# TheStageAI/TheWhisper

Hardware: AMD Instinct MI355X
Metric: transcription tokens/sec (node), whisper-large-v3 10s chunks (higher is better)
Workload: dtype f16

## Files before the change

### thewhisper_amd/csrc/api.hip

```cpp
#include "../../include/thewhisper.h"
#include "tw_common.h"

#include <algorithm>
#include <cmath>
#include <cstdarg>
#include <cstdio>
#include <cstring>
#include <map>
#include <mutex>
#include <set>
#include <chrono>
#include <string>
#include <tuple>
#include <vector>

namespace {

thread_local std::string g_create_error;

struct LayerW {
  void *ln1_g = nullptr, *ln1_b = nullptr;
  void *wqkv = nullptr, *bqkv = nullptr;
  unsigned char *s_qkv = nullptr, *s_o = nullptr, *s_qc = nullptr, *s_oc = nullptr, *s_1 = nullptr, *s_2 = nullptr;
  void *wo = nullptr, *bo = nullptr;
// ... 11 lines not shown

struct tw_ctx {
  tw_config cfg{};
  int dtype = 1;
  bool w8 = false;
  int a16 = 0;
  bool fuse_cq = false;
  bool enc_fold = true;
  float *ln_stats_a = nullptr, *ln_stats_b = nullptr;
  float* du = nullptr;
  float* dstats = nullptr;
  unsigned char* logit_ws = nullptr;
  size_t esz = 2;
  int d = 0, H = 0, ffn = 0, V = 0, T = 0, Tp = 0, P = 0, C = 0, Bmax = 0, Le = 0, Ld = 0, n_mels = 0, Ha = 0;
  std::string err;
  std::vector<void*> allocs;
  hipStream_t own_stream = nullptr;

  void *conv1_w = nullptr, *conv1_b = nullptr, *conv2_w = nullptr, *conv2_b = nullptr;
  void *enc_pos_raw = nullptr, *enc_pos = nullptr, *enc_ln_g = nullptr, *enc_ln_b = nullptr;
  void *tok_emb = nullptr, *dec_pos = nullptr, *dec_ln_g = nullptr, *dec_ln_b = nullptr;
  void* logit_w = nullptr;
  float *logit_gw = nullptr, *logit_cb = nullptr;
  std::vector<LayerW> enc, dec;
  std::set<std::string> loaded;
  bool finalized = false;
  bool shares_weights = false;

  LogmelTables lm{};
  float* logspec_ws = nullptr; size_t logspec_cap = 0;
  unsigned* lm_max = nullptr;
  int* n_valid_dev = nullptr;

  void *melT = nullptr, *h1 = nullptr, *xa = nullptr, *xb = nullptr, *lnbuf = nullptr, *qbuf = nullptr, *kbuf = nullptr,
       *vtbuf = nullptr, *attn = nullptr, *ffnh = nullptr, *enc_out = nullptr;
  int encoded_B = 0, cross_B = 0;

  void *self_k = nullptr, *self_v = nullptr, *cross_k = nullptr, *cross_v = nullptr;
  unsigned char *cross_ksc = nullptr, *cross_vsc = nullptr;
  void *dx0 = nullptr, *dx1 = nullptr, *dq = nullptr, *datt = nullptr, *dh = nullptr;
  float* logits = nullptr;
  float* align = nullptr;
  int* align_slot = nullptr;
  int *seq = nullptr, *cur_ids = nullptr, *finished = nullptr, *last_ts = nullptr;
  DecState* stt = nullptr;
  int* begin_suppress_dev = nullptr; int* suppress_dev = nullptr;
  SamplerPartial* sampler_partials = nullptr;
  float* sample_inv_t = nullptr; uint32_t* sample_key = nullptr; uint32_t* sample_off = nullptr; int* sample_noisy = nullptr;
  SamplePartial* sample_parts = nullptr;
  int* filter_top_k = nullptr; float* filter_top_p = nullptr; int* filter_choice = nullptr;
  unsigned* suppress_bits = nullptr;
  int* h_pinned = nullptr;
  int* row_ids = nullptr;
  int* h_rows = nullptr;
  int* row_lastts = nullptr;
  int* row_choice = nullptr;
  int* verify_state = nullptr;
  int* h_verify = nullptr;
  int* bias_tab = nullptr; int* h_bias = nullptr;
  int* repeat_tab = nullptr; int* h_repeat = nullptr;
  int* n_pad_tab = nullptr; int* h_n_pad = nullptr;
  int last_draft[4] = {0, 0, 0, 0};
  size_t row_ids_cap = 0;
  int* score_seq = nullptr;
  int *score_bsup = nullptr, *score_sup = nullptr;
  unsigned* score_bits = nullptr;
  ScorePartial* score_parts = nullptr;
  float* score_out = nullptr;
  float* h_score = nullptr;
  int row_cap = 0;
  int* h_stage = nullptr;
  size_t h_stage_ints = 0;
  hipEvent_t ring_ev[8]{};
  int last_seq_len = 0, last_n_prompt = 0;
  int dec_key_bound = 0;
  int enc_pos_rows = 0;

  float *zbuf = nullptr, *mat = nullptr, *out_ts = nullptr;
  signed char* trace = nullptr;
  int* n_cols = nullptr;

  std::map<std::string, hipGraphExec_t> step_graphs;
  std::string step_graph_key;

  hipEvent_t ev0[5]{}, ev1[5]{};
  bool ev_valid[5]{};
  int last_steps = 0;
};

namespace {

int fail(tw_ctx* c, int code, const char* fmt, ...) {
  char buf[512];
  va_list ap;
  va_start(ap, fmt);
  vsnprintf(buf, sizeof buf, fmt, ap);
  va_end(ap);
  if (c) c->err = buf; else g_create_error = buf;
  return code;
}

#define HIPCHK(c, expr)                                                                       \
  do {                                                                                        \
    hipError_t _e = (expr);                                                                   \
    if (_e != hipSuccess)                                                                     \
      return fail((c), TW_EHIP, "%s failed: %s (%s:%d)", #expr, hipGetErrorString(_e), __FILE__, __LINE__); \
  } while (0)

template <typename P>
int dalloc(tw_ctx* c, P** p, size_t bytes, bool zero) {
  void* q = nullptr;
  if (bytes == 0) bytes = 16;
  hipError_t e = hipMalloc(&q, bytes);
  if (e != hipSuccess) return fail(c, TW_ENOMEM, "hipMalloc(%zu) failed: %s", bytes, hipGetErrorString(e));
  c->allocs.push_back(q);
  if (zero) {
    e = hipMemset(q, 0, bytes);
    if (e != hipSuccess) return fail(c, TW_EHIP, "hipMemset failed: %s", hipGetErrorString(e));
  }
  *p = reinterpret_cast<P*>(q);
  return TW_OK;
}
#define ALLOC(c, ptr, bytes, zero)                   \
  do {                                               \
    int _r = dalloc((c), &(ptr), (bytes), (zero));   \
    if (_r != TW_OK) return _r;                      \
  } while (0)

inline hipStream_t pick_stream(tw_ctx* c, void* s) { return s ? reinterpret_cast<hipStream_t>(s) : c->own_stream; }

struct DeviceGuard {
  int prev = -1;
  bool switched = false;
  explicit DeviceGuard(int dev) {
    if (hipGetDevice(&prev) == hipSuccess && prev != dev) switched = hipSetDevice(dev) == hipSuccess;
  }
  ~DeviceGuard() {
    if (switched) (void)hipSetDevice(prev);
  }
  DeviceGuard(const DeviceGuard&) = delete;
  DeviceGuard& operator=(const DeviceGuard&) = delete;
};
#define TW_ON_DEVICE(c) DeviceGuard _tw_guard((c)->cfg.device)

char* at(void* base, size_t elems, size_t esz) { return reinterpret_cast<char*>(base) + elems * esz; }

void build_mel_bank(int n_mels, std::vector<float>& bank, std::vector<int>& lo, std::vector<int>& hi) {
  const int nb = 201;
  auto hz2mel = [](double f) { return f >= 1000.0 ? 15.0 + std::log(f / 1000.0) * (27.0 / std::log(6.4)) : 3.0 * f / 200.0; };
  auto mel2hz = [](double m) { return m >= 15.0 ? 1000.0 * std::exp((std::log(6.4) / 27.0) * (m - 15.0)) : 200.0 * m / 3.0; };
  const double mmin = hz2mel(0.0), mmax = hz2mel(8000.0);
  std::vector<double> ff(n_mels + 2);
  for (int i = 0; i < n_mels + 2; ++i) ff[i] = mel2hz(mmin + (mmax - mmin) * (double)i / (double)(n_mels + 1));
  bank.assign((size_t)nb * n_mels, 0.f);
  lo.assign(n_mels, nb);
  hi.assign(n_mels, 0);
  for (int k = 0; k < nb; ++k) {
    const double fk = 8000.0 * (double)k / (double)(nb - 1);
    for (int m = 0; m < n_mels; ++m) {
      const double down = -(ff[m] - fk) / (ff[m + 1] - ff[m]);
      const double up = (ff[m + 2] - fk) / (ff[m + 2] - ff[m + 1]);
      double v = std::fmax(0.0, std::fmin(down, up));
      v *= 2.0 / (ff[m + 2] - ff[m]);
      const float vf = (float)v;
      bank[(size_t)k * n_mels + m] = vf;
      if (vf != 0.f) {
        if (k < lo[m]) lo[m] = k;
        if (k + 1 > hi[m]) hi[m] = k + 1;
      }
    }
  }
  for (int m = 0; m < n_mels; ++m)
    if (hi[m] == 0) lo[m] = 0;
}

int upload(tw_ctx* c, void* dst, const void* src, size_t bytes) {
  HIPCHK(c, hipMemcpy(dst, src, bytes, hipMemcpyHostToDevice));
  return TW_OK;
}

void tic(tw_ctx* c, int i, hipStream_t st) { (void)hipEventRecord(c->ev0[i], st); }
void toc(tw_ctx* c, int i, hipStream_t st) { (void)hipEventRecord(c->ev1[i], st); c->ev_valid[i] = true; }

}

extern "C" {

const char* tw_version(void) { return TW_VERSION_STRING; }

const char* tw_last_error(const tw_ctx* ctx) { return ctx ? ctx->err.c_str() : g_create_error.c_str(); }

int tw_destroy(tw_ctx* c) {
  if (!c) return TW_OK;
  TW_ON_DEVICE(c);
  (void)hipDeviceSynchronize();
  for (auto& kv : c->step_graphs) (void)hipGraphExecDestroy(kv.second);
  for (void* p : c->allocs) (void)hipFree(p);
  if (c->h_pinned) (void)hipHostFree(c->h_pinned);
  if (c->h_stage) (void)hipHostFree(c->h_stage);
  if (c->h_rows) (void)hipHostFree(c->h_rows);
  if (c->h_verify) (void)hipHostFree(c->h_verify);
  if (c->h_score) (void)hipHostFree(c->h_score);
  if (c->h_bias) (void)hipHostFree(c->h_bias);
  if (c->h_repeat) (void)hipHostFree(c->h_repeat);
  if (c->h_n_pad) (void)hipHostFree(c->h_n_pad);
  for (int i = 0; i < 5; ++i) {
    if (c->ev0[i]) (void)hipEventDestroy(c->ev0[i]);
    if (c->ev1[i]) (void)hipEventDestroy(c->ev1[i]);
  }
  for (int i = 0; i < 8; ++i)
    if (c->ring_ev[i]) (void)hipEventDestroy(c->ring_ev[i]);
  if (c->own_stream) (void)hipStreamDestroy(c->own_stream);
  delete c;
  return TW_OK;
}

static int create_ctx(const tw_config* cfg, const tw_ctx* share, tw_ctx** out);

int tw_create(const tw_config* cfg, tw_ctx** out) { return create_ctx(cfg, nullptr, out); }

int tw_create_sibling(const tw_ctx* src, int32_t max_batch, tw_ctx** out) {
  if (!src || !out) return fail(nullptr, TW_EINVAL, "tw_create_sibling: null argument");
  if (!src->finalized) return fail(nullptr, TW_ESTATE, "tw_create_sibling: the source context's weights are not finalized");
  if (src->shares_weights) return fail(nullptr, TW_EINVAL, "tw_create_sibling: the source is itself a sibling (create it from the owner)");
  tw_config cfg = src->cfg;
  cfg.max_batch = max_batch;
  return create_ctx(&cfg, src, out);
}

static int create_ctx(const tw_config* cfg, const tw_ctx* share, tw_ctx** out) {
  if (!cfg || !out) return fail(nullptr, TW_EINVAL, "tw_create: null argument");
  *out = nullptr;
  if (cfg->heads <= 0 || cfg->d_model != cfg->heads * 64)
    return fail(nullptr, TW_EINVAL, "head_dim must be 64 (d_model=%d heads=%d)", cfg->d_model, cfg->heads);
  if (cfg->dtype != TW_BF16 && cfg->dtype != TW_F32 && cfg->dtype != TW_F16 && cfg->dtype != TW_BF16_MXFP8 && cfg->dtype != TW_BF16_W8A16)
    return fail(nullptr, TW_EINVAL, "dtype must be TW_BF16, TW_F16, TW_F32, TW_BF16_MXFP8 or TW_BF16_W8A16");
  const bool cfg_w8 = cfg->dtype == TW_BF16_MXFP8 || cfg->dtype == TW_BF16_W8A16;
  if (cfg_w8 && (cfg->d_model % 128 || cfg->ffn % 128))
    return fail(nullptr, TW_EINVAL, "TW_BF16_MXFP8 / TW_BF16_W8A16 need d_model and ffn to be multiples of 128");
  if (cfg->d_model % 64 || cfg->ffn % 64 || cfg->d_model > 1280)
    return fail(nullptr, TW_EINVAL, "d_model/ffn must be multiples of 64 and d_model <= 1280");
  if (cfg->max_batch < 1 || cfg->max_batch > 64) return fail(nullptr, TW_EINVAL, "max_batch must be in [1,64]");
  if (cfg->dtype == TW_BF16_MXFP8 && cfg->max_batch > 16)
    return fail(nullptr, TW_EINVAL, "TW_BF16_MXFP8: max_batch must be in [1,16] (TW_BF16_W8A16 takes up to 64 streams)");
  if (cfg->source_positions < 8 || cfg->source_positions > 1500 || cfg->target_positions < 8 || cfg->target_positions > 511)
    return fail(nullptr, TW_EINVAL, "source_positions must be in [8,1500], target_positions in [8,511]");
  if (cfg->n_align_heads < 0 || cfg->n_align_heads > TW_MAX_ALIGN_HEADS) return fail(nullptr, TW_EINVAL, "bad n_align_heads");
  if (cfg->n_mels < 1 || cfg->n_mels > 256) return fail(nullptr, TW_EINVAL, "bad n_mels");
  int ndev = 0;
  if (hipGetDeviceCount(&ndev) != hipSuccess || ndev <= 0)
    return fail(nullptr, TW_EHIP, "no HIP device available (the MI355X path has no CPU fallback)");
  if (cfg->device < 0 || cfg->device >= ndev) return fail(nullptr, TW_EINVAL, "device %d out of range", cfg->device);
  DeviceGuard guard(cfg->device);
  int cur = -1;
  if (hipGetDevice(&cur) != hipSuccess || cur != cfg->device) return fail(nullptr, TW_EHIP, "hipSetDevice(%d) failed", cfg->device);

  tw_ctx* c = new tw_ctx();
  c->cfg = *cfg;
  c->w8 = cfg_w8;
  c->a16 = cfg->dtype == TW_BF16_W8A16;
  c->dtype = c->w8 ? (int)TW_BF16 : cfg->dtype;
  c->esz = c->dtype == TW_F32 ? 4 : 2;
  c->d = cfg->d_model; c->H = cfg->heads; c->ffn = cfg->ffn; c->V = cfg->vocab;
  c->T = cfg->source_positions; c->Tp = (c->T + 63) / 64 * 64; c->P = cfg->target_positions;
  c->n_mels = cfg->n_mels; c->C = (cfg->n_mels + 63) / 64 * 64;
  c->Bmax = cfg->max_batch; c->Le = cfg->enc_layers; c->Ld = cfg->dec_layers; c->Ha = cfg->n_align_heads;
  c->fuse_cq = c->d == c->H * 64;
  c->enc_fold = c->d % 64 == 0 && c->d <= 1280;
  auto bail = [&](int r) { g_create_error = c->err; tw_destroy(c); return r; };
#define CALLOC(ptr, bytes, zero) do { int _r = dalloc(c, &(ptr), (bytes), (zero)); if (_r != TW_OK) return bail(_r); } while (0)
#define CHIP(expr) do { hipError_t _e = (expr); if (_e != hipSuccess) { fail(c, TW_EHIP, "%s: %s", #expr, hipGetErrorString(_e)); return bail(TW_EHIP); } } while (0)
  CHIP(hipStreamCreate(&c->own_stream));
  for (int i = 0; i < 5; ++i) { CHIP(hipEventCreate(&c->ev0[i])); CHIP(hipEventCreate(&c->ev1[i])); }
  for (int i = 0; i < 8; ++i) CHIP(hipEventCreateWithFlags(&c->ring_ev[i], hipEventDisableTiming));
  CHIP(hipHostMalloc(reinterpret_cast<void**>(&c->h_pinned), sizeof(int) * (8 * 64 + 64 + 16), hipHostMallocDefault));
  c->h_stage_ints = (size_t)c->Bmax * c->P + 3 * (size_t)c->Bmax + 64 + 1024 + 16 + 6 * 64 + 2 * 64;
  CHIP(hipHostMalloc(reinterpret_cast<void**>(&c->h_stage), sizeof(int) * c->h_stage_ints, hipHostMallocDefault));

  const size_t e = c->esz;
// ... 542 lines not shown
bool getenv_off_fuse() {
  static const bool off = []() { const char* e = getenv("TW_FUSE_CQ"); return e && atoi(e) == 0; }();
  return off;
}

int decode_core(tw_ctx* c, int B, hipStream_t st, int rs = 0, const int* ids = nullptr, bool embed = true, bool rows_logits = false,
                bool record_alignment = true, const int* n_pad = nullptr) {
  const int d = c->d, H = c->H, F = c->ffn, T = c->T, P = c->P, dt = c->dtype;
  const size_t e = c->esz;
  if (n_pad && (rs != 0 || !embed)) return fail(c, TW_EINVAL, "decode_core: a ragged step is an ordinary step with its own embedding");
  if (n_pad) HIPCHK(c, launch_embed_ragged(dt, c->cur_ids, c->stt, n_pad, c->tok_emb, c->dec_pos, c->dx0, B, d, st));
  else if (embed) HIPCHK(c, launch_embed(dt, rs > 0 ? ids : c->cur_ids, c->stt, c->tok_emb, c->dec_pos, c->dx0, B, d, rs, st));
  void* xin = c->dx0;
  void* xmid = c->dx1;
  const int Pp = (P + 63) / 64 * 64;
  const size_t self_layer = (size_t)c->Bmax * Pp * d;
  const size_t cross_layer = (size_t)c->Bmax * c->Tp * d;
  for (int l = 0; l < c->Ld; ++l) {
    const LayerW& L = c->dec[l];
    void* sk = at(c->self_k, self_layer * l, e);
    void* sv = at(c->self_v, self_layer * l, e);
    const bool fq_on = c->fuse_cq && !getenv_off_fuse() && d / (L.tr_o ? L.tr_o : 16) <= 192;
    {
      GemvArgs a{};
      a.x = xin; a.ldx = d; a.ln_gw = L.qkv_gw; a.ln_cb = L.qkv_cb; a.W = L.wqkv; a.wscale = L.s_qkv; a.a16 = c->a16; a.N = (fq_on ? 4 : 3) * d; a.K = d; a.B = B;
      a.y = c->dq; a.ldy = d; a.kcache = sk; a.vcache = sv; a.cache_bstride = (long long)Pp * d; a.cache_hstride = (long long)Pp * 64; a.d_model = d; a.stt = c->stt;
      a.u = fq_on ? c->du : nullptr;
      a.rows_streams = rs;
      a.n_pad = n_pad;
      HIPCHK(c, launch_gemv(dt, a, st));
    }
    if (n_pad) HIPCHK(c, launch_dec_self_attn_ragged(dt, c->dq, sk, sv, Pp, c->datt, B, H, c->dec_key_bound > 0 ? c->dec_key_bound : P, c->stt, n_pad, st));
    else HIPCHK(c, launch_dec_self_attn(dt, c->dq, sk, sv, Pp, c->datt, B, H, c->dec_key_bound > 0 ? c->dec_key_bound : P, c->stt, rs, st));
    {
      GemvArgs a{};
      a.x = c->datt; a.ldx = d; a.W = L.wo; a.wscale = L.s_o; a.a16 = c->a16; a.tr = L.tr_o; a.bias = L.bo; a.N = (fq_on ? 2 : 1) * d; a.K = d; a.B = B;
      a.res = xin; a.ldres = d; a.y = xmid; a.ldy = d;
      if (fq_on) { a.u = c->du; a.nsplit = d; a.stats = c->dstats; }
      HIPCHK(c, launch_gemv(dt, a, st));
    }
    FusedQ fq{};
    if (fq_on) {
      fq.u = c->du; fq.stats = c->dstats; fq.n_part = d / (L.tr_o ? L.tr_o : 16); fq.gw = L.qc_gw; fq.cb = L.qc_cb; fq.d = d;
    } else {
      GemvArgs a{};
      a.x = xmid; a.ldx = d; a.ln_gw = L.qc_gw; a.ln_cb = L.qc_cb; a.W = L.wq_c; a.wscale = L.s_qc; a.a16 = c->a16; a.tr = L.tr_qc; a.N = d; a.K = d; a.B = B;
      a.y = c->dq; a.ldy = d;
      HIPCHK(c, launch_gemv(dt, a, st));
    }
    HIPCHK(c, launch_dec_cross_attn(dt, c->dq, fq, at(c->cross_k, cross_layer * l, c->w8 ? 1 : e), at(c->cross_v, cross_layer * l, c->w8 ? 1 : e),
                                    c->datt, B, H, T, c->Tp, (c->Ha > 0 && record_alignment) ? c->align_slot + (size_t)l * H : nullptr, c->align,
                                    record_alignment ? c->Ha : 0,
                                    P, c->stt, c->w8 ? c->cross_ksc + (size_t)c->Bmax * H * c->Tp * l : nullptr,
                                    c->w8 ? c->cross_vsc + (size_t)c->Bmax * H * c->Tp * l : nullptr, rs, st));
    {
      GemvArgs a{};
      a.x = c->datt; a.ldx = d; a.W = L.wo_c; a.wscale = L.s_oc; a.a16 = c->a16; a.tr = L.tr_oc; a.bias = L.bo_c; a.N = d; a.K = d; a.B = B; a.res = xmid; a.ldres = d;
      a.y = xin; a.ldy = d;
      HIPCHK(c, launch_gemv(dt, a, st));
    }
    {
      GemvArgs a{};
      a.x = xin; a.ldx = d; a.ln_gw = L.fc1_gw; a.ln_cb = L.fc1_cb; a.W = L.w1; a.wscale = L.s_1; a.a16 = c->a16; a.tr = L.tr_1; a.N = F; a.K = d; a.B = B;
      a.gelu = 1; a.y = c->dh; a.ldy = F;
      HIPCHK(c, launch_gemv(dt, a, st));
    }
    {
      GemvArgs a{};
      a.x = c->dh; a.ldx = F; a.W = L.w2; a.wscale = L.s_2; a.a16 = c->a16; a.tr = L.tr_2; a.bias = L.b2; a.N = d; a.K = F; a.B = B; a.res = xin; a.ldres = d;
      a.y = xmid; a.ldy = d;
      HIPCHK(c, launch_gemv(dt, a, st));
    }
    void* t = xin; xin = xmid; xmid = t;
  }
  if (rs == 0 || rows_logits) {
    GemvArgs a{};
    a.x = xin; a.ldx = d; a.ln_gw = c->logit_gw; a.ln_cb = c->logit_cb; a.W = c->logit_w; a.wscale = c->logit_ws; a.a16 = c->a16; a.N = c->V; a.K = d; a.B = B;
    a.y_f32 = c->logits;
    HIPCHK(c, launch_gemv(dt, a, st));
  }
  return TW_OK;
}

int prefill_core(tw_ctx* c, int B, const int* tok, int ld, int n_pos, hipStream_t st) {
  if (n_pos <= 0) return TW_OK;
  const int cap = (c->w8 && !c->a16) ? 16 : 64;
  if (B > cap) return fail(c, TW_EINVAL, "prefill: %d streams exceed the %d rows of a launch", B, cap);
  const int L = std::max(1, std::min(cap, c->row_cap) / B);
  if ((size_t)n_pos * B > c->row_ids_cap) return fail(c, TW_EINVAL, "prefill: %d positions x %d streams exceed the row table", n_pos, B);
  int* h = c->h_rows;
  for (int p = 0; p < n_pos; ++p)
    for (int b = 0; b < B; ++b) h[(size_t)p * B + b] = tok[(size_t)b * ld + p];
  HIPCHK(c, hipMemcpyAsync(c->row_ids, h, sizeof(int) * (size_t)n_pos * B, hipMemcpyHostToDevice, st));
  for (int p0 = 0; p0 < n_pos; p0 += L) {
    const int l = std::min(L, n_pos - p0);
    c->dec_key_bound = std::min(((p0 + l + 63) / 64) * 64, ((c->P + 63) / 64) * 64);
    int r = decode_core(c, l * B, st, B, c->row_ids + (size_t)p0 * B);
    if (r != TW_OK) return r;
    HIPCHK(c, launch_advance(c->stt, l, st));
  }
  return TW_OK;
}

int verify_round(tw_ctx* c, int B, int* tok, int ld, int n_begin, int ts_begin, int p_start, int p_end, int rows_cap, const SamplerArgs& sa0,
                 hipStream_t st, int* p_next, int* n_launches, int p_given, int* next_given, const SeqBiasArgs* ba,
                 const RepeatArgs* ra) {
  const int n_pos = p_end - p_start + 1;
  if (n_pos < 1 || B > rows_cap) return fail(c, TW_EINVAL, "verify: bad round [%d, %d] for %d streams", p_start, p_end, B);
  if ((size_t)n_pos * B > c->row_ids_cap) return fail(c, TW_EINVAL, "verify: %d positions x %d streams exceed the row table", n_pos, B);
  const int L = std::max(1, rows_cap / B);
  int* h = c->h_rows;
  int* hl = c->h_rows + c->row_ids_cap;
  for (int b = 0; b < B; ++b) {
    int lt = -1;
    for (int p = n_begin; p < p_start; ++p) if (tok[(size_t)b * ld + p] >= ts_begin) lt = tok[(size_t)b * ld + p];
    for (int p = p_start; p <= p_end; ++p) {
      const int t = tok[(size_t)b * ld + p];
      if (p >= n_begin && t >= ts_begin) lt = t;
      h[(size_t)(p - p_start) * B + b] = t;
      hl[(size_t)(p - p_start) * B + b] = lt;
    }
  }
  int* hv = c->h_verify;
  hv[66] = 0x7fffffff; hv[67] = 0;
  HIPCHK(c, hipMemcpyAsync(c->row_ids, h, sizeof(int) * (size_t)n_pos * B, hipMemcpyHostToDevice, st));
  HIPCHK(c, hipMemcpyAsync(c->row_lastts, hl, sizeof(int) * (size_t)n_pos * B, hipMemcpyHostToDevice, st));
  HIPCHK(c, hipMemcpyAsync(c->verify_state, hv + 66, sizeof(int) * 2, hipMemcpyHostToDevice, st));
  for (int p0 = p_start; p0 <= p_end; p0 += L) {
    const int l = std::min(L, p_end - p0 + 1);
    const size_t off = (size_t)(p0 - p_start) * B;
    c->dec_key_bound = std::min(((p0 + l + 63) / 64) * 64, ((c->P + 63) / 64) * 64);
    int r = decode_core(c, l * B, st, B, c->row_ids + off, true, true);
    if (r != TW_OK) return r;
    SamplerArgs sa = sa0;
    sa.B = l * B; sa.rows_streams = B; sa.row_pos0 = p0; sa.row_lastts = c->row_lastts + off; sa.row_choice = c->row_choice + off;
    sa.row_last_pos = p_end; sa.row_is_last = (p0 + l > p_end) ? 1 : 0; sa.verify_state = c->verify_state;
    if (ba) {
      SeqBiasArgs b = *ba;
      b.rows = l * B; b.rows_streams = B; b.row_pos0 = p0;
      HIPCHK(c, launch_seq_bias(b, st));
    }
    if (ra) {
      RepeatArgs rp = *ra;
      rp.rows = l * B; rp.rows_streams = B; rp.row_pos0 = p0;
      HIPCHK(c, launch_repeat(rp, st));
    }
    HIPCHK(c, launch_sampler_rows(sa, st));
    HIPCHK(c, hipMemcpyAsync(hv, c->verify_state, sizeof(int) * (2 + B), hipMemcpyDeviceToHost, st));
    HIPCHK(c, hipStreamSynchronize(st));
    ++*n_launches;
    if (hv[1] != 0) {
      const int pn = hv[1];
      if (pn < p0 + 1 || pn > p0 + l) return fail(c, TW_EHIP, "verify: decided position %d outside the launch [%d, %d)", pn - 1, p0, p0 + l);
      bool same = pn <= p_given;
      for (int b = 0; b < B; ++b) {
        same = same && tok[(size_t)b * ld + pn] == hv[2 + b];
        tok[(size_t)b * ld + pn] = hv[2 + b];
      }
      *next_given = same ? 1 : 0;
      *p_next = pn;
      return TW_OK;
    }
  }
  return fail(c, TW_EHIP, "verify: the round ended without a decision");
}

constexpr size_t kSeqBiasTabWords = kSeqBiasHeader + 2 * (size_t)TW_BIAS_MAX_SEQS + 2 * ((size_t)TW_BIAS_MAX_SEQS + 1) + TW_BIAS_MAX_TOKENS;

int pack_seq_bias(tw_ctx* c, int B, const tw_bias_opts* bo, std::vector<int>& tab) {
  const char* fn = "tw_generate_greedy_biased";
  const int S = bo->n_seq;
  if (S < 0 || S > TW_BIAS_MAX_SEQS) return fail(c, TW_EINVAL, "%s: %d sequences (at most %d)", fn, S, TW_BIAS_MAX_SEQS);
  if (!bo->row_off || !bo->seq_off || !bo->tokens || !bo->bias) return fail(c, TW_EINVAL, "%s: null array in tw_bias_opts", fn);
  if (bo->row_off[0] != 0 || bo->row_off[B] != S) return fail(c, TW_EINVAL, "%s: row_off must run from 0 to n_seq", fn);
  for (int b = 0; b < B; ++b)
    if (bo->row_off[b + 1] < bo->row_off[b]) return fail(c, TW_EINVAL, "%s: row_off decreases at row %d", fn, b);
  if (bo->seq_off[0] != 0) return fail(c, TW_EINVAL, "%s: seq_off must start at 0", fn);
  for (int i = 0; i < S; ++i) {
    const long long L = (long long)bo->seq_off[i + 1] - bo->seq_off[i];
    if (L < 1 || L > TW_BIAS_MAX_SEQ_LEN) return fail(c, TW_EINVAL, "%s: sequence %d has %lld tokens (1 .. %d)", fn, i, L, TW_BIAS_MAX_SEQ_LEN);
    if (bo->seq_off[i + 1] > TW_BIAS_MAX_TOKENS) return fail(c, TW_EINVAL, "%s: more than %d tokens", fn, TW_BIAS_MAX_TOKENS);
    if (!std::isfinite(bo->bias[i])) return fail(c, TW_EINVAL, "%s: the bias of sequence %d is NaN or infinite", fn, i);
  }
// ... 37 lines not shown
  auto append = [&](int slot, const int* p, size_t n) { tab[slot] = (int)tab.size(); tab.insert(tab.end(), p, p + n); };
  append(0, grp_off.data(), grp_off.size());
  append(1, grp_tok.data(), grp_tok.size());
  append(2, seq_off.data(), seq_off.size());
  append(3, reinterpret_cast<const int*>(bias.data()), bias.size());
  append(4, tokens.data(), tokens.size());
  if (tab.size() > kSeqBiasTabWords) return fail(c, TW_EINVAL, "%s: the packed table exceeds its capacity", fn);
  return TW_OK;
}

int pack_repeat(tw_ctx* c, const char* fn, int rows, int max_n, const tw_repeat_opts* ro, int* tab, bool* any) {
  if (rows < 1 || rows > 64) return fail(c, TW_EINVAL, "%s: %d rows (1..64)", fn, rows);
  if (ro->penalty_ignore < 0) return fail(c, TW_EINVAL, "%s: penalty_ignore %d < 0", fn, ro->penalty_ignore);
  *any = false;
  for (int b = 0; b < 64; ++b) {
    const float r = (b < rows && ro->penalty) ? ro->penalty[b] : 1.0f;
    const int N = (b < rows && ro->no_repeat_ngram) ? ro->no_repeat_ngram[b] : 0;
    if (!std::isfinite(r) || !(r > 0.f)) return fail(c, TW_EINVAL, "%s: the penalty of row %d is NaN, infinite or <= 0", fn, b);
    if (N < 0 || N > max_n) return fail(c, TW_EINVAL, "%s: no_repeat_ngram[%d] = %d outside [0, %d]", fn, b, N, max_n);
    memcpy(tab + b, &r, sizeof r);
    tab[64 + b] = N;
    *any |= r != 1.0f || N != 0;
  }
  tab[128] = ro->penalty_ignore;
  for (int i = 129; i < kRepeatTabWords; ++i) tab[i] = 0;
  return TW_OK;
}

int reset_state(tw_ctx* c, int n_prompt, hipStream_t st) {
  DecState s{0, n_prompt, 0, 0};
  memcpy(c->h_pinned + 576, &s, sizeof s);
  HIPCHK(c, hipMemcpyAsync(c->stt, c->h_pinned + 576, sizeof s, hipMemcpyHostToDevice, st));
  return TW_OK;
}

}

extern "C" {

int tw_decoder_reset(tw_ctx* c, int32_t B, void* stream) {
  if (!c) return TW_EINVAL;
  TW_ON_DEVICE(c);
  if (B < 1 || B > c->cross_B) return fail(c, TW_ESTATE, "tw_decoder_reset: B=%d but cross K/V holds %d clips", B, c->cross_B);
  hipStream_t st = pick_stream(c, stream);
  int r = reset_state(c, 0, st);
  if (r != TW_OK) return r;
  c->dec_key_bound = c->P;
  HIPCHK(c, hipStreamSynchronize(st));
  return TW_OK;
}

int tw_decode_step(tw_ctx* c, int32_t B, const int32_t* ids_host, float* logits_dev, void* stream) {
  if (!c || !ids_host) return fail(c, TW_EINVAL, "tw_decode_step: null argument");
  TW_ON_DEVICE(c);
  if (B < 1 || B > c->cross_B) return fail(c, TW_ESTATE, "tw_decode_step: B=%d but cross K/V holds %d clips", B, c->cross_B);
  hipStream_t st = pick_stream(c, stream);
  HIPCHK(c, hipMemcpyAsync(c->cur_ids, ids_host, sizeof(int) * B, hipMemcpyHostToDevice, st));
  int r = decode_core(c, B, st);
  if (r != TW_OK) return r;
  if (logits_dev)
    HIPCHK(c, hipMemcpyAsync(logits_dev, c->logits, sizeof(float) * (size_t)B * c->V, hipMemcpyDeviceToDevice, st));
  HIPCHK(c, launch_advance(c->stt, 1, st));
  return TW_OK;
}

static int generate_loop(tw_ctx* c, int32_t B, const int32_t* prompt, int32_t n_prompt, const tw_greedy_opts* o, const tw_sample_opts* so,
                         const tw_filter_opts* fo, const tw_bias_opts* bo, int32_t* out_ids, int32_t* out_len, void* stream,
                         const int32_t* n_pad = nullptr, const tw_repeat_opts* ro = nullptr) {
  const char* fn = n_pad ? "tw_generate_greedy_ragged" : ro ? "tw_generate_greedy_repeat" : bo ? "tw_generate_greedy_biased" : fo ? "tw_generate_sample_filtered" : so ? "tw_generate_sample" : "tw_generate_greedy";
  const bool ragged = n_pad != nullptr;
  if (ragged && (so || fo || bo || ro || o->n_forced != 0 || o->n_draft != 0)) return fail(c, TW_EINVAL, "%s: padding goes with the plain greedy call only", fn);
  if (B < 1 || B > c->cross_B) return fail(c, TW_ESTATE, "%s: B=%d but cross K/V holds %d clips", fn, B, c->cross_B);
  if (n_prompt < 1 || n_prompt >= c->P) return fail(c, TW_EINVAL, "bad n_prompt %d", n_prompt);
  if (o->n_begin_suppress > 64 || o->n_suppress > 1024) return fail(c, TW_EINVAL, "suppress lists too long");
  if (o->want_alignment && c->Ha == 0) return fail(c, TW_EINVAL, "want_alignment but the context has no alignment heads");
  const int n_forced = o->n_forced;
  if (n_forced < 0 || n_forced >= n_prompt) return fail(c, TW_EINVAL, "bad n_forced %d (n_prompt %d)", n_forced, n_prompt);
  const int n_draft = o->n_draft;
  if (n_draft < 0 || n_draft >= n_prompt || (n_draft > 0 && n_forced > 0))
    return fail(c, TW_EINVAL, "bad n_draft %d (n_prompt %d, n_forced %d: one of the two)", n_draft, n_prompt, n_forced);
  if (o->pad_id < 0 || o->pad_id >= c->V || o->eos_id < 0 || o->eos_id >= c->V)
    return fail(c, TW_EINVAL, "pad_id %d / eos_id %d outside the vocabulary", o->pad_id, o->eos_id);
  const int n_begin = n_prompt - n_forced - n_draft;
  int max_len = n_begin + o->max_new_tokens;
  if (o->max_length > 0 && o->max_length < max_len) max_len = o->max_length;
  if (max_len > c->P) max_len = c->P;
  if (max_len <= n_prompt) return fail(c, TW_EINVAL, "nothing to generate (max_len %d <= n_prompt %d)", max_len, n_prompt);
  const int out_ld = o->max_length > 0 ? o->max_length : max_len;
  const bool biased = bo != nullptr;
  std::vector<int> bias_tab;
  if (biased) {
    if (B > 64) return fail(c, TW_EINVAL, "%s: %d streams (1..64)", fn, B);
    int r = pack_seq_bias(c, B, bo, bias_tab);
    if (r != TW_OK) return r;
  }
  int repeat_tab[kRepeatTabWords];
  bool repeat = false;
  if (ro) {
    if (so || fo) return fail(c, TW_EINVAL, "%s: repeat options go with the greedy call only", fn);
    int r = pack_repeat(c, fn, B, c->P, ro, repeat_tab, &repeat);
    if (r != TW_OK) return r;
  }
  c->dec_key_bound = max_len;
  hipStream_t st = pick_stream(c, stream);
  const int P = c->P;

  int* hseq = c->h_stage;
  int* first = hseq + (size_t)c->Bmax * P;
  int* zeros = first + c->Bmax;
  int* neg = zeros + c->Bmax;
  int* bsup = neg + c->Bmax;
  int* sup = bsup + 64;
  DecState* s0p = reinterpret_cast<DecState*>(sup + 1024);
  float* h_inv_t = reinterpret_cast<float*>(sup + 1024 + 16);
  uint32_t* h_key = reinterpret_cast<uint32_t*>(h_inv_t + 64);
  uint32_t* h_off = h_key + 128;
  int* h_noisy = reinterpret_cast<int*>(h_off + 128);
  int* h_top_k = h_noisy + 64;
  float* h_top_p = reinterpret_cast<float*>(h_top_k + 64);
  for (size_t i = 0; i < (size_t)B * P; ++i) hseq[i] = o->pad_id;
  for (int b = 0; b < B; ++b) {
    for (int i = 0; i < n_prompt; ++i) {
      const int t = prompt[(size_t)b * n_prompt + i];
      if (t < 0 || t >= c->V) return fail(c, TW_EINVAL, "prompt token %d out of range", t);
      hseq[(size_t)b * P + i] = t;
    }
    first[b] = prompt[(size_t)b * n_prompt + (n_forced > 0 ? n_prompt - 1 : 0)];
    zeros[b] = (so && so->temperature[b] < 0.f) ? 1 : 0;
    neg[b] = -1;
    if (so) {
      const float t = so->temperature[b];
      h_noisy[b] = t > 0.f ? 1 : 0;
      h_inv_t[b] = t > 0.f ? 1.0f / t : 1.0f;
      const uint64_t sd = so->seed ? so->seed[b] : 0, of = so->offset ? so->offset[b] : 0;
      h_key[2 * b] = (uint32_t)sd; h_key[2 * b + 1] = (uint32_t)(sd >> 32);
      h_off[2 * b] = (uint32_t)of; h_off[2 * b + 1] = (uint32_t)(of >> 32);
      if (fo) {
        h_top_k[b] = (t > 0.f && fo->top_k) ? fo->top_k[b] : 0;
        h_top_p[b] = (t > 0.f && fo->top_p) ? fo->top_p[b] : 1.0f;
      }
    }
    for (int i = n_begin; i < n_prompt; ++i) {
      const int t = prompt[(size_t)b * n_prompt + i];
      if (t == o->eos_id) return fail(c, TW_EINVAL, n_draft > 0 ? "a draft token is <eos>" : "a forced token is <eos>");
      if (n_forced > 0 && o->timestamps && t > o->no_timestamps_id) neg[b] = t;
    }
  }
  if (biased) {
    if (!c->bias_tab) ALLOC(c, c->bias_tab, sizeof(int) * kSeqBiasTabWords, false);
    if (!c->h_bias) HIPCHK(c, hipHostMalloc(reinterpret_cast<void**>(&c->h_bias), sizeof(int) * kSeqBiasTabWords));
    memcpy(c->h_bias, bias_tab.data(), sizeof(int) * bias_tab.size());
    HIPCHK(c, hipMemcpyAsync(c->bias_tab, c->h_bias, sizeof(int) * bias_tab.size(), hipMemcpyHostToDevice, st));
  }
  if (repeat) {
    if (!c->repeat_tab) ALLOC(c, c->repeat_tab, sizeof(int) * kRepeatTabWords, true);
    if (!c->h_repeat) HIPCHK(c, hipHostMalloc(reinterpret_cast<void**>(&c->h_repeat), sizeof(int) * kRepeatTabWords));
    memcpy(c->h_repeat, repeat_tab, sizeof repeat_tab);
    HIPCHK(c, hipMemcpyAsync(c->repeat_tab, c->h_repeat, sizeof repeat_tab, hipMemcpyHostToDevice, st));
  }
  if (ragged) {
    if (!c->n_pad_tab) ALLOC(c, c->n_pad_tab, sizeof(int) * 64, true);
    if (!c->h_n_pad) HIPCHK(c, hipHostMalloc(reinterpret_cast<void**>(&c->h_n_pad), sizeof(int) * 64));
    for (int b = 0; b < 64; ++b) c->h_n_pad[b] = b < B ? n_pad[b] : 0;
    HIPCHK(c, hipMemcpyAsync(c->n_pad_tab, c->h_n_pad, sizeof(int) * 64, hipMemcpyHostToDevice, st));
  }
  HIPCHK(c, hipMemcpyAsync(c->seq, hseq, sizeof(int) * (size_t)B * P, hipMemcpyHostToDevice, st));
  HIPCHK(c, hipMemcpyAsync(c->cur_ids, first, sizeof(int) * B, hipMemcpyHostToDevice, st));
  HIPCHK(c, hipMemcpyAsync(c->finished, zeros, sizeof(int) * B, hipMemcpyHostToDevice, st));
  HIPCHK(c, hipMemcpyAsync(c->last_ts, neg, sizeof(int) * B, hipMemcpyHostToDevice, st));
  if (so) {
    HIPCHK(c, hipMemcpyAsync(c->sample_inv_t, h_inv_t, sizeof(float) * B, hipMemcpyHostToDevice, st));
    HIPCHK(c, hipMemcpyAsync(c->sample_key, h_key, sizeof(uint32_t) * 2 * B, hipMemcpyHostToDevice, st));
    HIPCHK(c, hipMemcpyAsync(c->sample_off, h_off, sizeof(uint32_t) * 2 * B, hipMemcpyHostToDevice, st));
    HIPCHK(c, hipMemcpyAsync(c->sample_noisy, h_noisy, sizeof(int) * B, hipMemcpyHostToDevice, st));
  }
  if (fo) {
    HIPCHK(c, hipMemcpyAsync(c->filter_top_k, h_top_k, sizeof(int) * B, hipMemcpyHostToDevice, st));
    HIPCHK(c, hipMemcpyAsync(c->filter_top_p, h_top_p, sizeof(float) * B, hipMemcpyHostToDevice, st));
  }
  if (o->n_begin_suppress > 0) {
    memcpy(bsup, o->begin_suppress, sizeof(int) * o->n_begin_suppress);
    HIPCHK(c, hipMemcpyAsync(c->begin_suppress_dev, bsup, sizeof(int) * o->n_begin_suppress, hipMemcpyHostToDevice, st));
  }
  if (o->n_suppress > 0) {
    memcpy(sup, o->suppress, sizeof(int) * o->n_suppress);
    HIPCHK(c, hipMemcpyAsync(c->suppress_dev, sup, sizeof(int) * o->n_suppress, hipMemcpyHostToDevice, st));
  }
  HIPCHK(c, launch_suppress_bitmap(c->suppress_dev, o->n_suppress, c->suppress_bits, c->V, st));
  *s0p = DecState{0, n_begin, max_len - 1, B};
  HIPCHK(c, hipMemcpyAsync(c->stt, s0p, sizeof(DecState), hipMemcpyHostToDevice, st));
  int s_start = n_forced > 0 ? n_prompt - 1 : 0;
  if (n_forced > 0) {
    int r = prefill_core(c, B, prompt, n_prompt, s_start, st);
    if (r != TW_OK) return r;
  }

  SamplerArgs sa{};
  sa.logits = c->logits; sa.V = c->V; sa.B = B; sa.seq = c->seq; sa.seq_ld = P; sa.cur_ids = c->cur_ids;
  sa.finished = c->finished; sa.last_ts = c->last_ts; sa.stt = c->stt;
  sa.eos = o->eos_id; sa.pad = o->pad_id; sa.min_new = o->min_new_tokens; sa.timestamps = o->timestamps;
  sa.no_ts_id = o->no_timestamps_id; sa.max_initial_ts = o->max_initial_timestamp_index;
  sa.begin_suppress = c->begin_suppress_dev; sa.n_begin_suppress = o->n_begin_suppress;
  sa.suppress_bits = c->suppress_bits; sa.partials = c->sampler_partials;
  SeqBiasArgs ba{};
  ba.logits = c->logits; ba.V = c->V; ba.rows = B; ba.seq = c->seq; ba.seq_ld = P; ba.finished = c->finished; ba.stt = c->stt; ba.tab = c->bias_tab;
  RepeatArgs rpa{};
  rpa.logits = c->logits; rpa.V = c->V; rpa.rows = B; rpa.seq = c->seq; rpa.seq_ld = P; rpa.finished = c->finished; rpa.stt = c->stt; rpa.tab = c->repeat_tab;
  c->last_draft[0] = n_draft * B; c->last_draft[1] = c->last_draft[2] = c->last_draft[3] = 0;
  bool draft_all_done = false;
  if (n_draft > 0) {
    constexpr int first_rows = 64, retry_rows = 16, max_rounds = 16;
    const int cap = std::min((c->w8 && !c->a16) ? 16 : 64, c->row_cap);
    if (B > cap) return fail(c, TW_EINVAL, "n_draft: %d streams exceed the %d rows of a launch", B, cap);
    const int ts_begin = o->timestamps ? o->no_timestamps_id + 1 : c->V;
    const int p_end = n_prompt - 1;
    tic(c, 3, st);
    int pos = 0, rounds = 0;
    while (true) {
      const int rows = rounds == 0 ? std::min(cap, std::max(first_rows, B)) : std::min(cap, std::max(retry_rows, 4 * B));
      const int pe = rounds == 0 ? p_end : std::min(p_end, pos + std::max(1, rows / B) - 1);
      int pn = 0, next_given = 0;
      int r = verify_round(c, B, hseq, P, n_begin, ts_begin, pos, pe, rows, sa, st, &pn, &c->last_draft[2], p_end, &next_given, biased ? &ba : nullptr,
                           repeat ? &rpa : nullptr);
      if (r != TW_OK) return r;
      ++rounds;
      const int confirmed = pn - 1 - std::max(pos, n_begin - 1) + ((next_given && pn >= n_begin) ? 1 : 0);
      c->last_draft[1] += std::max(0, confirmed) * B;
      pos = pn;
      draft_all_done = true;
      bool any_done = false;
      for (int b = 0; b < B; ++b) {
        const bool done = pos >= n_begin && hseq[(size_t)b * P + pos] == o->eos_id;
        draft_all_done &= done;
        any_done |= done;
      }
      if (any_done || pos > p_end - 1 || pos >= max_len - 1 || rounds >= max_rounds || (rounds > 1 && confirmed <= 0)) break;
    }
    c->last_draft[3] = rounds;
    s_start = pos;
  }
  sa.tok_emb = c->tok_emb; sa.pos_emb = c->dec_pos; sa.x_next = ragged ? nullptr : c->dx0; sa.d = c->d; sa.dtype = c->dtype;
  const int* pad_tab = ragged ? c->n_pad_tab : nullptr;
  if (!ragged) HIPCHK(c, launch_embed(c->dtype, c->cur_ids, c->stt, c->tok_emb, c->dec_pos, c->dx0, B, c->d, 0, st));

  char keybuf[256];
  snprintf(keybuf, sizeof keybuf, "%d|%d|%d|%d|%d|%d|%d|%d|%d|%c", B, o->eos_id, o->pad_id, o->min_new_tokens, o->timestamps,
           o->no_timestamps_id, o->max_initial_timestamp_index, o->n_begin_suppress, o->n_suppress, ragged ? 'r' : repeat ? (biased ? 'q' : 'p') : biased ? 'b' : fo ? 'f' : so ? 's' : 'g');
  SampleArgs sma{};
  sma.inv_t = c->sample_inv_t; sma.key = c->sample_key; sma.off = c->sample_off; sma.noisy = c->sample_noisy; sma.parts = c->sample_parts;
  FilterArgs fla{};
  fla.top_k = c->filter_top_k; fla.top_p = c->filter_top_p; fla.choice = c->filter_choice;
  auto sample_step = [&]() -> hipError_t {
    if (biased) {
      hipError_t e = launch_seq_bias(ba, st);
      if (e != hipSuccess) return e;
    }
    if (repeat) {
      hipError_t e = launch_repeat(rpa, st);
      if (e != hipSuccess) return e;
    }
    if (!so) return launch_sampler(sa, st);
    sma.s = sa;
    if (!fo) return launch_sample(sma, st);
    fla.sm = sma;
    return launch_sample_filtered(fla, st);
  };
  const bool use_graph = c->cfg.use_graph != 0;
  if (use_graph && c->step_graph_key != keybuf) {
    for (auto& kv : c->step_graphs) (void)hipGraphExecDestroy(kv.second);
    c->step_graphs.clear();
    c->step_graph_key = keybuf;
  }
  auto graph_for = [&](int kb, int n, hipGraphExec_t* out) -> int {
    const std::string k = std::to_string(kb) + "x" + std::to_string(n);
    auto it = c->step_graphs.find(k);
    if (it != c->step_graphs.end()) { *out = it->second; return TW_OK; }
    hipGraph_t g = nullptr;
    c->dec_key_bound = kb;
    HIPCHK(c, hipStreamBeginCapture(st, hipStreamCaptureModeThreadLocal));
    int r = TW_OK;
    hipError_t es = hipSuccess;
    for (int i = 0; i < n && r == TW_OK && es == hipSuccess; ++i) {
      r = decode_core(c, B, st, 0, nullptr, ragged, false, true, pad_tab);
      if (r == TW_OK) es = sample_step();
    }
    hipError_t ee = hipStreamEndCapture(st, &g);
    if (r != TW_OK) { if (g) (void)hipGraphDestroy(g); return r; }
    if (es != hipSuccess || ee != hipSuccess) {
      if (g) (void)hipGraphDestroy(g);
      return fail(c, TW_EHIP, "decode-step graph capture failed: %s", hipGetErrorString(es != hipSuccess ? es : ee));
    }
    hipGraphExec_t ex = nullptr;
    hipError_t ei = hipGraphInstantiate(&ex, g, nullptr, nullptr, 0);
    (void)hipGraphDestroy(g);
    if (ei != hipSuccess) return fail(c, TW_EHIP, "hipGraphInstantiate failed: %s", hipGetErrorString(ei));
    c->step_graphs[k] = ex;
    *out = ex;
    return TW_OK;
  };

  static const bool host_timing = getenv("TW_HOST_TIMING") != nullptr;
  const auto ht0 = std::chrono::steady_clock::now();
  auto ht_ms = [&]() { return std::chrono::duration<double, std::milli>(std::chrono::steady_clock::now() - ht0).count(); };
  double ht_first = 0, ht_loop = 0;
  if (n_draft == 0) tic(c, 3, st);
  constexpr int group = 2;
  constexpr int group_forced = 8;
  const int LAG = std::max(1, 4 / group);
  int steps = 0, launches = 0;
  bool all_done = draft_all_done;
  for (int s = s_start; s < max_len - 1 && !all_done;) {
    const bool eos_free = use_graph && launches >= 1 && group_forced > group && s + group_forced <= max_len - 1 &&
                          s + group_forced - 1 < n_begin + o->min_new_tokens - 1;
    const int n = eos_free ? group_forced : ((use_graph && s + group <= max_len - 1) ? group : 1);
    const int last = s + n - 1;
    const int kb = std::min(((last + 64) / 64) * 64, ((max_len + 63) / 64) * 64);
    if (use_graph) {
      hipGraphExec_t ex = nullptr;
      int r = graph_for(kb, n, &ex);
      if (r != TW_OK) return r;
      HIPCHK(c, hipGraphLaunch(ex, st));
    } else {
      c->dec_key_bound = kb;
      int r = decode_core(c, B, st, 0, nullptr, ragged, false, true, pad_tab);
      if (r != TW_OK) return r;
      HIPCHK(c, sample_step());
    }
    steps += n;
    s += n;
    const int slot = launches % 8;
    HIPCHK(c, hipMemcpyAsync(c->h_pinned + slot * 64, c->finished, sizeof(int) * B, hipMemcpyDeviceToHost, st));
    HIPCHK(c, hipEventRecord(c->ring_ev[slot], st));
    if (launches >= LAG) {
      const int ps = (launches - LAG) % 8;
      HIPCHK(c, hipEventSynchronize(c->ring_ev[ps]));
      bool done = true;
      for (int b = 0; b < B; ++b) done &= (c->h_pinned[ps * 64 + b] != 0);
      all_done = done;
    }
    if (launches == 0) ht_first = ht_ms();
    ++launches;
  }
  toc(c, 3, st);
  ht_loop = ht_ms();
  c->last_steps = steps;
  HIPCHK(c, hipMemcpyAsync(hseq, c->seq, sizeof(int) * (size_t)B * P, hipMemcpyDeviceToHost, st));
  HIPCHK(c, hipStreamSynchronize(st));
  if (host_timing) {
    float dev_ms = 0.f;
    (void)hipEventElapsedTime(&dev_ms, c->ev0[3], c->ev1[3]);
    fprintf(stderr, "TW_HOST_TIMING generate B=%d steps=%d launches=%d: first launch submitted at %.3f ms, host loop done at %.3f ms, "
                    "synchronised at %.3f ms; device loop (events) %.3f ms\n", B, steps, launches, ht_first, ht_loop, ht_ms(), dev_ms);
  }

  const int produced = s_start + steps + 1;
  const int scan_from = n_draft > 0 ? std::max(s_start, n_begin) : n_prompt;
  int L = scan_from + 1;
  for (int b = 0; b < B; ++b) {
    if (so && so->temperature[b] < 0.f) continue;
    int lb = produced;
    for (int i = scan_from; i < produced; ++i)
      if (hseq[(size_t)b * P + i] == o->eos_id) { lb = i + 1; break; }
    if (lb > L) L = lb;
  }
  for (int b = 0; b < B; ++b) {
    bool ended = false;
    for (int i = 0; i < out_ld; ++i) {
      int v = o->pad_id;
      if (i < L) {
        v = hseq[(size_t)b * P + i];
        if (ended) v = o->pad_id;
        if (i >= scan_from && v == o->eos_id) ended = true;
      }
      out_ids[(size_t)b * out_ld + i] = v;
    }
  }
  *out_len = L;
  c->last_seq_len = L;
  c->last_n_prompt = n_prompt;
  return TW_OK;
}

int tw_generate_greedy(tw_ctx* c, int32_t B, const int32_t* prompt, int32_t n_prompt, const tw_greedy_opts* o,
                       int32_t* out_ids, int32_t* out_len, void* stream) {
  if (!c || !prompt || !o || !out_ids || !out_len) return fail(c, TW_EINVAL, "tw_generate_greedy: null argument");
  TW_ON_DEVICE(c);
  return generate_loop(c, B, prompt, n_prompt, o, nullptr, nullptr, nullptr, out_ids, out_len, stream);
}

int tw_generate_greedy_biased(tw_ctx* c, int32_t B, const int32_t* prompt, int32_t n_prompt, const tw_greedy_opts* o, const tw_bias_opts* bo,
                              int32_t* out_ids, int32_t* out_len, void* stream) {
  if (!c || !prompt || !o || !out_ids || !out_len) return fail(c, TW_EINVAL, "tw_generate_greedy_biased: null argument");
  TW_ON_DEVICE(c);
  return generate_loop(c, B, prompt, n_prompt, o, nullptr, nullptr, (bo && bo->n_seq != 0) ? bo : nullptr, out_ids, out_len, stream);
}

int tw_generate_greedy_repeat(tw_ctx* c, int32_t B, const int32_t* prompt, int32_t n_prompt, const tw_greedy_opts* o, const tw_bias_opts* bo,
                              const tw_repeat_opts* ro, int32_t* out_ids, int32_t* out_len, void* stream) {
  if (!c || !prompt || !o || !out_ids || !out_len) return fail(c, TW_EINVAL, "tw_generate_greedy_repeat: null argument");
  TW_ON_DEVICE(c);
  if (ro && B > 64) return fail(c, TW_EINVAL, "tw_generate_greedy_repeat: %d streams (1..64)", B);
  return generate_loop(c, B, prompt, n_prompt, o, nullptr, nullptr, (bo && bo->n_seq != 0) ? bo : nullptr, out_ids, out_len, stream, nullptr, ro);
}

int tw_generate_greedy_ragged(tw_ctx* c, int32_t B, const int32_t* prompt, int32_t n_prompt, const tw_greedy_opts* o, const int32_t* n_pad,
                              int32_t* out_ids, int32_t* out_len, void* stream) {
  const char* fn = "tw_generate_greedy_ragged";
  if (!c || !prompt || !o || !out_ids || !out_len) return fail(c, TW_EINVAL, "%s: null argument", fn);
  TW_ON_DEVICE(c);
  bool padded = false;
  if (B > 64) return fail(c, TW_EINVAL, "%s: %d streams (1..64)", fn, B);
  if (n_pad) {
    for (int b = 0; b < B; ++b) {
      if (n_pad[b] < 0 || n_pad[b] >= n_prompt)
        return fail(c, TW_EINVAL, "%s: n_pad[%d] = %d outside [0, n_prompt = %d)", fn, b, n_pad[b], n_prompt);
      padded |= n_pad[b] > 0;
    }
  }
  if (!padded) return generate_loop(c, B, prompt, n_prompt, o, nullptr, nullptr, nullptr, out_ids, out_len, stream);
  if (o->n_forced != 0 || o->n_draft != 0)
    return fail(c, TW_EINVAL, "%s: n_forced %d / n_draft %d: forced and draft tokens do not go with padded rows", fn, o->n_forced, o->n_draft);
  return generate_loop(c, B, prompt, n_prompt, o, nullptr, nullptr, nullptr, out_ids, out_len, stream, n_pad);
}

static int generate_sample_checked(const char* fn, tw_ctx* c, int32_t B, const int32_t* prompt, int32_t n_prompt, const tw_greedy_opts* o,
                                   const tw_sample_opts* so, const tw_filter_opts* fo, int32_t* out_ids, int32_t* out_len, void* stream) {
  if (!c || !prompt || !o || !so || !so->temperature || !so->seed || !out_ids || !out_len)
    return fail(c, TW_EINVAL, "%s: null argument", fn);
// ... 461 lines not shown
```

Before: 11690.

## Prefill plain prompts in batched row launches and capture prefill as HIP graph

Measured after the change: 11760, median of 6. Within noise of the previous version (+0.6%).

```diff
diff --git a/thewhisper_amd/csrc/api.hip b/thewhisper_amd/csrc/api.hip
--- a/thewhisper_amd/csrc/api.hip
+++ b/thewhisper_amd/csrc/api.hip
@@ -117,6 +117,7 @@
 
   std::map<std::string, hipGraphExec_t> step_graphs;
   std::string step_graph_key;
+  std::map<std::string, hipGraphExec_t> prefill_graphs;
 
   hipEvent_t ev0[5]{}, ev1[5]{};
   bool ev_valid[5]{};
@@ -230,6 +231,7 @@
   TW_ON_DEVICE(c);
   (void)hipDeviceSynchronize();
   for (auto& kv : c->step_graphs) (void)hipGraphExecDestroy(kv.second);
+  for (auto& kv : c->prefill_graphs) (void)hipGraphExecDestroy(kv.second);
   for (void* p : c->allocs) (void)hipFree(p);
   if (c->h_pinned) (void)hipHostFree(c->h_pinned);
   if (c->h_stage) (void)hipHostFree(c->h_stage);
@@ -938,9 +940,11 @@
   return TW_OK;
 }
 
+int prefill_rows_cap(const tw_ctx* c) { return (c->w8 && !c->a16) ? 16 : 64; }
+
 int prefill_core(tw_ctx* c, int B, const int* tok, int ld, int n_pos, hipStream_t st) {
   if (n_pos <= 0) return TW_OK;
-  const int cap = (c->w8 && !c->a16) ? 16 : 64;
+  const int cap = prefill_rows_cap(c);
   if (B > cap) return fail(c, TW_EINVAL, "prefill: %d streams exceed the %d rows of a launch", B, cap);
   const int L = std::max(1, std::min(cap, c->row_cap) / B);
   if ((size_t)n_pos * B > c->row_ids_cap) return fail(c, TW_EINVAL, "prefill: %d positions x %d streams exceed the row table", n_pos, B);
@@ -948,13 +952,36 @@
   for (int p = 0; p < n_pos; ++p)
     for (int b = 0; b < B; ++b) h[(size_t)p * B + b] = tok[(size_t)b * ld + p];
   HIPCHK(c, hipMemcpyAsync(c->row_ids, h, sizeof(int) * (size_t)n_pos * B, hipMemcpyHostToDevice, st));
-  for (int p0 = 0; p0 < n_pos; p0 += L) {
-    const int l = std::min(L, n_pos - p0);
-    c->dec_key_bound = std::min(((p0 + l + 63) / 64) * 64, ((c->P + 63) / 64) * 64);
-    int r = decode_core(c, l * B, st, B, c->row_ids + (size_t)p0 * B);
-    if (r != TW_OK) return r;
-    HIPCHK(c, launch_advance(c->stt, l, st));
-  }
+  auto launches = [&]() -> int {
+    for (int p0 = 0; p0 < n_pos; p0 += L) {
+      const int l = std::min(L, n_pos - p0);
+      c->dec_key_bound = std::min(((p0 + l + 63) / 64) * 64, ((c->P + 63) / 64) * 64);
+      int r = decode_core(c, l * B, st, B, c->row_ids + (size_t)p0 * B);
+      if (r != TW_OK) return r;
+      HIPCHK(c, launch_advance(c->stt, l, st));
+    }
+    return TW_OK;
+  };
+  if (c->cfg.use_graph == 0) return launches();
+  const std::string k = std::to_string(B) + "x" + std::to_string(n_pos);
+  auto it = c->prefill_graphs.find(k);
+  if (it == c->prefill_graphs.end()) {
+    hipGraph_t g = nullptr;
+    HIPCHK(c, hipStreamBeginCapture(st, hipStreamCaptureModeThreadLocal));
+    const int r = launches();
+    const hipError_t ee = hipStreamEndCapture(st, &g);
+    if (r != TW_OK) { if (g) (void)hipGraphDestroy(g); return r; }
+    if (ee != hipSuccess) {
+      if (g) (void)hipGraphDestroy(g);
+      return fail(c, TW_EHIP, "prefill graph capture failed: %s", hipGetErrorString(ee));
+    }
+    hipGraphExec_t ex = nullptr;
+    const hipError_t ei = hipGraphInstantiate(&ex, g, nullptr, nullptr, 0);
+    (void)hipGraphDestroy(g);
+    if (ei != hipSuccess) return fail(c, TW_EHIP, "hipGraphInstantiate failed: %s", hipGetErrorString(ei));
+    it = c->prefill_graphs.emplace(k, ex).first;
+  }
+  HIPCHK(c, hipGraphLaunch(it->second, st));
   return TW_OK;
 }
 
@@ -1158,6 +1185,8 @@
   if (o->pad_id < 0 || o->pad_id >= c->V || o->eos_id < 0 || o->eos_id >= c->V)
     return fail(c, TW_EINVAL, "pad_id %d / eos_id %d outside the vocabulary", o->pad_id, o->eos_id);
   const int n_begin = n_prompt - n_forced - n_draft;
+  const bool prompt_rows = !ragged && n_forced == 0 && n_draft == 0 && n_prompt >= 2 && B <= prefill_rows_cap(c);
+  const bool prefilled = n_forced > 0 || prompt_rows;
   int max_len = n_begin + o->max_new_tokens;
   if (o->max_length > 0 && o->max_length < max_len) max_len = o->max_length;
   if (max_len > c->P) max_len = c->P;
@@ -1201,7 +1230,7 @@
       if (t < 0 || t >= c->V) return fail(c, TW_EINVAL, "prompt token %d out of range", t);
       hseq[(size_t)b * P + i] = t;
     }
-    first[b] = prompt[(size_t)b * n_prompt + (n_forced > 0 ? n_prompt - 1 : 0)];
+    first[b] = prompt[(size_t)b * n_prompt + (prefilled ? n_prompt - 1 : 0)];
     zeros[b] = (so && so->temperature[b] < 0.f) ? 1 : 0;
     neg[b] = -1;
     if (so) {
@@ -1265,8 +1294,9 @@
   HIPCHK(c, launch_suppress_bitmap(c->suppress_dev, o->n_suppress, c->suppress_bits, c->V, st));
   *s0p = DecState{0, n_begin, max_len - 1, B};
   HIPCHK(c, hipMemcpyAsync(c->stt, s0p, sizeof(DecState), hipMemcpyHostToDevice, st));
-  int s_start = n_forced > 0 ? n_prompt - 1 : 0;
-  if (n_forced > 0) {
+  int s_start = prefilled ? n_prompt - 1 : 0;
+  if (n_draft == 0) tic(c, 3, st);
+  if (prefilled) {
     int r = prefill_core(c, B, prompt, n_prompt, s_start, st);
     if (r != TW_OK) return r;
   }
@@ -1379,7 +1409,6 @@
   const auto ht0 = std::chrono::steady_clock::now();
   auto ht_ms = [&]() { return std::chrono::duration<double, std::milli>(std::chrono::steady_clock::now() - ht0).count(); };
   double ht_first = 0, ht_loop = 0;
-  if (n_draft == 0) tic(c, 3, st);
   constexpr int group = 2;
   constexpr int group_forced = 8;
   const int LAG = std::max(1, 4 / group);
@@ -1419,7 +1448,7 @@
   }
   toc(c, 3, st);
   ht_loop = ht_ms();
-  c->last_steps = steps;
+  c->last_steps = steps + (prompt_rows ? s_start : 0);
   HIPCHK(c, hipMemcpyAsync(hseq, c->seq, sizeof(int) * (size_t)B * P, hipMemcpyDeviceToHost, st));
   HIPCHK(c, hipStreamSynchronize(st));
   if (host_timing) {
```
